# rubencart/NES-img-captioning

Hardware: AMD Instinct MI355X
Metric: population-members evaluated/sec (fc_caption, pop=512) at 1/2/4/8 GPUs (higher is better)
Workload: dtype fp32

## Files before the change

include/nicnes.h:

```cpp
#ifndef NICNES_H
#define NICNES_H

#include <stdint.h>

#ifdef __cplusplus
extern "C" {
#endif

#define NICNES_OK 0
#define NICNES_ERR_INVALID 1
#define NICNES_ERR_UNSUPPORTED 2
#define NICNES_ERR_HIP 3
#define NICNES_ERR_NOMEM 4
#define NICNES_ERR_FAULT 5

typedef struct nicnes_handle nicnes_handle;

typedef struct nicnes_config {
    int32_t vocab_size;
    int32_t input_encoding_size;
    int32_t rnn_size;
    int32_t fc_feat_size;
    int32_t seq_length;
    int32_t max_batch;
// ... 111 lines not shown
int nicnes_set_timing(nicnes_handle* h, int on);
int nicnes_kernel_times(nicnes_handle* h, float* out2_host);

int nicnes_decode_phase_times(nicnes_handle* h, float* out8_host);

int nicnes_set_decode_split(nicnes_handle* h, int32_t S, int32_t G);
int nicnes_decode_shape(nicnes_handle* h, int32_t B, int32_t count, int32_t* out3_host);
int nicnes_set_decode_streams(nicnes_handle* h, int32_t n);
int nicnes_set_decode_coop(nicnes_handle* h, int32_t mode);

int nicnes_sum_sensitivity(nicnes_handle* h, int32_t rows, float underflow, float* out_dev, void* stream);
int nicnes_decode_path(nicnes_handle* h, int32_t B, int32_t count, int32_t* out_host);
int nicnes_last_decode_lse(nicnes_handle* h, int32_t* bounded_host);
int nicnes_set_decode_screen(nicnes_handle* h, int32_t mode);
int nicnes_screen_stats(nicnes_handle* h, int64_t* out2_host);
int nicnes_test_logit_chain(nicnes_handle* h, uint64_t iteration, int32_t member, float sigma, int32_t sign,
                            const float* h_rows_dev, float* out_mfma_dev, float* out_chain_dev, void* stream);
int nicnes_test_certify_items(nicnes_handle* h, uint64_t iteration, int32_t member, float sigma, int32_t sign,
                              const float* h_rows_dev, const int32_t* items_host, int32_t n_items, float* out_dev,
                              void* stream);
int nicnes_test_certify_items_owned(nicnes_handle* h, uint64_t iteration, int32_t member, float sigma, int32_t sign,
                                    int32_t owner_by_id, const float* h_rows_dev, const int32_t* items_host,
                                    int32_t n_items, float* out_dev, void* stream);
int nicnes_test_score_rows(nicnes_handle* h, const int32_t* seq_dev, int32_t n_cand, int32_t rows,
                           const int32_t* member_batch_host, const float* lp_dev, const double* base_dev,
                           double* scores_out_dev, double* fitness_out_dev, void* stream);

int nicnes_es_create(nicnes_handle* h, int32_t max_parents, int32_t max_elites);
int nicnes_es_free(nicnes_handle* h);
int nicnes_es_set_mutation(nicnes_handle* h, int32_t mode);
// ... 27 lines not shown
```

nes-img-captioning_amd/csrc/decode_kernel.h:

```cpp
#pragma once
#define SCR_SLOTS (64 + 64 + 64 + 1 + 64)
#define PART_FLOATS (8 * 7 * 64)
#define COOP_CTR_STRIDE 32
#define SCREEN_CAP_WORDS(V1) ((size_t)(((V1) + 63) / 64) * 512)
#include <hip/hip_runtime.h>
#include <stdint.h>

struct DecodeParams {
    const float* theta;
    const float* noise;
    const uint64_t* noise_idx;
    const float* fc;
    const int32_t* member_batch;
    int32_t* seq;
    float* lp;
    const double* sample_u;
    float* scratch;
    int32_t* stats;
    float* slog;
    int32_t* slog_slots;
    int32_t slog_ns;
    int32_t* alive;
    int32_t* alive2;
    float* part;
// ... 10 lines not shown
    int32_t B_img;
    int32_t sign_off;
    int32_t rpi;
    int32_t G;
    int32_t S;
    int32_t alive_stride;
    int64_t D;
    int64_t off_img_w, off_img_b, off_emb_w, off_log_w, off_log_b, off_i2h_w, off_i2h_b, off_h2h_w, off_h2h_b;
};

struct ScreenArgs {
    uint32_t* cap;
    float* norm;
    float scale;
    unsigned long long* ctr;
};

struct MutHead {
    const float* head_noise;
    const uint64_t* head_idx;
    const float* mut_vec;
    int32_t mode;
};

struct ParentArgs {
    const float* parents;
    const int32_t* parent_of;
    int64_t stride;
};

#define DK_IMG 0
// ... 26 lines not shown
```

nes-img-captioning_amd/csrc/decode_kernel.hip:

```cpp
#include <hip/hip_runtime.h>
#include <stdint.h>

#include "../../include/nicnes_math.h"
#include "decode_kernel.h"

typedef float f32x4 __attribute__((ext_vector_type(4)));
typedef float f32x16 __attribute__((ext_vector_type(16)));
typedef unsigned u32x4 __attribute__((ext_vector_type(4)));
typedef __bf16 bf16x4 __attribute__((ext_vector_type(4)));
typedef __bf16 bf16x8 __attribute__((ext_vector_type(8)));
typedef __amdgpu_buffer_rsrc_t rsrc_t;

#define NTHREADS 512
#define LDS_ROW 132
#define SIGN_FLOATS (32 * LDS_ROW)
#define STAGE_FLOATS (2 * SIGN_FLOATS + 64)
#define STAGE64_FLOATS (2 * 64 * LDS_ROW + 128)
#define BF_ROW 68
#define BF_SIGN (64 * BF_ROW)
#define LOG2E 1.44269504088896340736f
#define H_SLOT_BYTES (4u * 64u * 64u)
#define NEG_INF (-__builtin_inff())

#ifndef DECODE_ABLATE
// ... 276 lines not shown
                                                const Stage64Regs& r) {
    float* b = buf + o.so;
#pragma unroll
    for (int u = 0; u < 4; ++u) {
        const f32x4 delta = r.z[u];
        *reinterpret_cast<f32x4*>(b + 16 * u * LDS_ROW) = r.w[u] + delta;
        *reinterpret_cast<f32x4*>(b + (64 + 16 * u) * LDS_ROW) = r.w[u] - delta;
    }
    if (bias) {
        const float delta = r.bz;
        const float v = o.bslot >= 64 ? r.bw - delta : r.bw + delta;
        buf[2 * 64 * LDS_ROW + o.bslot] = (o.bslot & 63) < valid ? v : NEG_INF;
    }
}

__device__ __forceinline__ void mfma_stage64(const float* w, const float* bias, const float (&Bop)[64], int lane,
                                             f32x16& acc0, f32x16& acc1) {
    const int hh = lane >> 5;
    const float* row0 = w + (lane & 31) * LDS_ROW + hh * 16;
    const float* row1 = row0 + 32 * LDS_ROW;
    acc0 = bias_init(bias, hh);
    acc1 = bias_init(bias + 32, hh);
#pragma unroll
    for (int T = 0; T < 4; ++T) {
        f32x4 a0[4], a1[4];
#pragma unroll
        for (int c = 0; c < 4; ++c) {
            a0[c] = *reinterpret_cast<const f32x4*>(row0 + T * 32 + 4 * c);
            a1[c] = *reinterpret_cast<const f32x4*>(row1 + T * 32 + 4 * c);
        }
// ... 697 lines not shown
    float acc = sgn ? bw - bz : bw + bz;
#pragma unroll
    for (int T = 0; T < 4; ++T) {
#pragma unroll
        for (int c = 0; c < 4; ++c) {
            const uint32_t ko = 4u * (uint32_t)(32 * T + 8 * c);
            const f32x4 w0 = ld4(theta_r, wo + ko), z0 = ld4(noise_r, wo + ko);
            const f32x4 w1 = ld4(theta_r, wo + ko + 16u), z1 = ld4(noise_r, wo + ko + 16u);
            const f32x4 a0 = sgn ? w0 - z0 : w0 + z0, a1 = sgn ? w1 - z1 : w1 + z1;
            acc = chain_chunk(acc, a0, a1, scr_r, row_lo, T, c);
        }
    }
    return acc;
}

__device__ __forceinline__ bool screen_scan(rsrc_t cap, uint32_t vo, int nst, float thr, float* lds, int tid, int& cnt,
                                            int& ncand) {
    uint32_t* list = reinterpret_cast<uint32_t*>(lds) + tid * SCREEN_HIT_CAP;
    int hits = 0;
    cnt = 0;
    for (int s0 = 0; s0 < nst; s0 += 16) {
        uint32_t wd[16];
#pragma unroll
        for (int j = 0; j < 16; ++j)
            wd[j] = __builtin_amdgcn_raw_buffer_load_b32(cap, (int)vo, (int)(2048u * (uint32_t)min(s0 + j, nst - 1)), 0);
#pragma unroll
        for (int j = 0; j < 16; ++j) {
            const uint32_t word = wd[j];
            if (s0 + j < nst && __builtin_bit_cast(float, word & ~31u) >= thr) {
                hits += (word & 16u) ? 4 : 1;
                ncand += (word & 16u) ? 32 : 2;
                if (cnt < SCREEN_HIT_CAP) list[cnt] = ((uint32_t)(s0 + j) << 8) | (word & 31u);
                ++cnt;
            }
        }
    }
    return hits <= SCREEN_HIT_CAP;
}

struct ListItems {
    const uint32_t* list;
    int cnt, hh, V1;
    template <class F>
    __device__ __forceinline__ void operator()(F&& f) const {
        for (int k = 0; k < cnt; ++k) {
            const uint32_t e = list[k];
            const int s = (int)(e >> 8), pr = (int)(e & 15u);
            const bool crowded = (e & 16u) != 0;
            const int i0 = crowded ? 0 : 2 * pr, i1 = crowded ? 32 : 2 * pr + 2;
            for (int i = i0; i < i1; ++i) {
                const int a = i & 15;
                const int v = 64 * s + 32 * (i >> 4) + 4 * hh + (a & 3) + 8 * (a >> 2);
// ... 37 lines not shown
__device__ __forceinline__ void cert_load_bias(const DecodeParams& p, rsrc_t theta_r, rsrc_t noise_r, const uint32_t* iw,
                                               int nv, float& bw, float& bz) {
    const uint32_t v = iw[min(lane_fresh() & 31, nv - 1)] & CERT_ID_MASK;
    const uint32_t bo = 4u * ((uint32_t)p.off_log_b + v);
    bw = ld1(theta_r, bo);
    bz = ld1(noise_r, bo);
}
__device__ __forceinline__ void cert_store(float* tile, int sgn, int T, const CertRegs& r) {
    const int lane = lane_fresh(), q = lane & 7;
    float* b = tile + (lane >> 3) * LDS_ROW + T * 32 + (q & 1) * 16 + 4 * (q >> 1);
#pragma unroll
    for (int u = 0; u < 4; ++u)
        *reinterpret_cast<f32x4*>(b + 8 * u * LDS_ROW) = sgn ? r.w[u] - r.z[u] : r.w[u] + r.z[u];
}

template <class Each, class Sink>
__device__ __forceinline__ void certify_tiles(const DecodeParams& p, rsrc_t theta_r, rsrc_t noise_r, int sgn,
                                              const float (&hB)[64], float* lds, int tid, int n_mine, const Each& each,
                                              Sink&& sink, int pm) {
    const int lane = tid & 63, hh = lane >> 5;
    const int wave = __builtin_amdgcn_readfirstlane(tid >> 6);
    float* tile = lds + CERT_WAVE_AT + wave * CERT_WAVE_FLOATS;
    float* bias = tile + SIGN_FLOATS;
    uint32_t* items = reinterpret_cast<uint32_t*>(bias + 32);
    int inc = n_mine;
#pragma unroll
    for (int d = 1; d < 64; d <<= 1) {
        const int u = __shfl_up(inc, d);
        inc += lane >= d ? u : 0;
    }
    const int total = __builtin_amdgcn_readlane(inc, 63), first = inc - n_mine;
    __syncthreads();
#if DECODE_PROF
    if (pm >= 0 && total == 0 && lane == 0)
        p.seq[(size_t)(blockIdx.x * gridDim.y + blockIdx.y) * 4096 + CERT_PROF_WAVE_AT((pm - 1 - 640) / 5 - 1) + wave] = 0;
#endif
    for (int b0 = 0; b0 < total; b0 += CERT_ITEMS) {
        const int nb = min(CERT_ITEMS, total - b0);
        const bool mine = first < b0 + nb && first + n_mine > b0;
        if (mine) {
            int pos = first - b0;
            each([&](int v) {
                if ((unsigned)pos < (unsigned)nb) items[pos] = ((uint32_t)lane << CERT_ID_BITS) | (uint32_t)v;
                ++pos;
            });
        }
        wave_lds_order();
// ... 65 lines not shown
    }
}

__global__ __launch_bounds__(NTHREADS) void nicnes_screen_norm_kernel(DecodeParams p, ScreenArgs sa) {
    __shared__ float red[4][8];
#include "screen_norm_body.inc"
}

__global__ __launch_bounds__(NTHREADS) void nicnes_screen_norm_es_kernel(DecodeParams p0, ParentArgs pa, ScreenArgs sa) {
    __shared__ float red[4][8];
    DecodeParams p = p0;
    p.theta = pa.parents + (int64_t)pa.parent_of[blockIdx.x] * pa.stride;
#include "screen_norm_body.inc"
}

template <int G, bool PAIRS, bool PEEL = true, class Tail = NoTail, class Hook = NoHook>
__device__ __forceinline__ void logit_stages(float* lds, const DecodeParams& p, uint64_t nidx, int wave, int sgn,
                                             int hf, const float (&hB)[64], int s0, int s1, RowState& st,
                                             Stage64Regs& s64, bool preloaded = false, Tail&& tail = Tail(),
                                             const Hook& hook = Hook()) {
    const rsrc_t lw_r = make_rsrc(p.theta + p.off_log_w, 4u * 128u * (uint32_t)p.V1);
    const rsrc_t lz_r = make_rsrc(p.noise + nidx + p.off_log_w, 4u * 128u * (uint32_t)p.V1);
    const rsrc_t lbw_r = make_rsrc(p.theta + p.off_log_b, 4u * (uint32_t)p.V1);
    const rsrc_t lbz_r = make_rsrc(p.noise + nidx + p.off_log_b, 4u * (uint32_t)p.V1);
    auto lsrc = [&](int s) {
        StageSrc Sx;
        Sx.w_r = lw_r; Sx.z_r = lz_r; Sx.b_r = lbw_r; Sx.bz_r = lbz_r;
        Sx.so_a = 32768u * (uint32_t)s; Sx.so_b = Sx.so_a + 16384u;
        Sx.bso = 256u * (uint32_t)s; Sx.bda = 0u; Sx.bdb = 128u;
        Sx.valid = p.V1 - 64 * s;
        return Sx;
    };
    const LaneOffs lo = lane_offs(wave, 128u);
    LaneOffsBf lob{0, 0};
    if constexpr (Hook::bf) lob = lane_offs_bf(wave);
    const int hh = lane_fresh() >> 5, vl = 4 * hh + (G == 4 ? 0 : 32 * hf);
    const bool bias = wave < 2;
    if (!preloaded) stage64_load_o(lsrc(s0), lo, bias, s64);
    auto sstore = [&](float* buf, int valid) __attribute__((always_inline)) {
        if constexpr (Hook::bf) stage64_store_bf(buf, valid, lo, lob.sob, bias, s64);
        else stage64_store_o(buf, valid, lo, bias, s64);
    };
    sstore(lds, lsrc(s0).valid);
    if (PEEL) stage64_load_o(lsrc(min(s0 + 1, s1 - 1)), lo, bias, s64);
    else if (s0 + 1 < s1) stage64_load_o(lsrc(s0 + 1), lo, bias, s64);
    __syncthreads();
    f32x16 a0, a1, b0, b1;
#pragma unroll
    for (int r = 0; r < 16; ++r) { b0[r] = NEG_INF; b1[r] = NEG_INF; }
    auto stage = [&](auto mode_t, int s, f32x16& o0, f32x16& o1, const f32x16& q0, const f32x16& q1) {
        constexpr int MODE = decltype(mode_t)::value;
        const int sn = min(s + 1, s1 - 1);
        const float* buf = lds + ((s - s0) & 1) * STAGE64_FLOATS;
        const float* wsg = buf + sgn * (Hook::bf ? BF_SIGN : 64 * LDS_ROW);
        const float* bsg = buf + 2 * (Hook::bf ? BF_SIGN : 64 * LDS_ROW) + 64 * sgn;
        auto mid = [&]() __attribute__((always_inline)) {
#if !(DECODE_ABLATE & 2)
            if constexpr (MODE == 0) {
                sstore(lds + ((s - s0 + 1) & 1) * STAGE64_FLOATS, lsrc(sn).valid);
                stage64_load_o(lsrc(min(s + 2, s1 - 1)), lo, bias, s64);
            } else if constexpr (MODE == 1) {
// ... 286 lines not shown
            for (int i = 0; i < 64; ++i) Bb[i >> 3][i & 7] = (__bf16)hB[i];
            const ScreenStage ss{scap_r, 4u * (uint32_t)(c.wave * 64 + lane_fresh()), 2.0f * seps + SCREEN_HU_MAX, Bb, st};
            logit_stages<4, true, true>(lds, p, nidx, c.wave, c.sgn, 0, hB, 0, nl, st, s64, pre, tail, ss);
        } else {
            logit_stages<4, PAIRS>(lds, p, nidx, c.wave, c.sgn, 0, hB, 0, nl, st, s64, pre, tail);
        }
        cell_pre = xpre;
        PROF_MARK(120 + 24 * (t + 1));

        const float m_o = __shfl_xor(st.m, 32);
        const float s_o = __shfl_xor(st.s, 32);
        float m = fmaxf(st.m, m_o);
        float stot = st.s * __builtin_amdgcn_exp2f((st.m - m) * LOG2E) + s_o * __builtin_amdgcn_exp2f((m_o - m) * LOG2E);
        TieWindow w = tie_window(stot, PAIRS, SCREEN ? p.lse_margin + 2.0f * seps : p.lse_margin);
        bool sforce = false;
        float lse = w.lse;
        int tok = 0x7fffffff;
        float lp_tok = 0.f;
        bool amb = false;
        if constexpr (SAMPLE) {
            const double u = u_pre;
            const float mo = __shfl_xor(sm, 32), ro = __shfl_xor(sref, 32);
            const double To = __shfl_xor(sT, 32);
            const float mr = fmaxf(sm, mo), R = fmaxf(sref, ro);
            const double ta = samp_scale(sT, sref - R), tb = samp_scale(To, ro - R);
            const double T = c.hh == 0 ? ta + tb : tb + ta;
            const float lse_s = (float)(log(T) + (double)R * 0.69314718055994531 - (double)mr);
            const uint32_t vo = 16u * (uint32_t)c.lane + SLOG_WAVE_BYTES * (uint32_t)c.wave;
#if DECODE_ABLATE & 512
            tok = 1 + (int)(u * 9000.0);
            lp_tok = -lse_s;
#else
            if (p.force_exact)
                sample_pick<true>(p, c.slog_r, vo, c.hh, mr, lse_s, R, u * T, tok, lp_tok);
            else
                sample_pick<false>(p, c.slog_r, vo, c.hh, mr, lse_s, R, u * T, tok, lp_tok, 120 + 24 * (t + 1));
#endif
        } else {
            if constexpr (SCREEN) {
                const float d = 2.0f * seps + w.hu_out;
                const float thr = (m - d) - SCREEN_PACK_REL * (fabsf(m) + d);
                const bool need = unf_prev != 0.f || p.no_mask;
                bool bad = p.force_exact || !(fabsf(thr) < 3.0e38f) || !(w.hu_out <= SCREEN_HU_MAX) || !(stot > 0.f);
                st.r1v = st.r0v = st.ev = NEG_INF;
                st.r1i = st.r0i = 0x7fffffff;
                int ncand = 0, ccnt = 0;
                if (need && !bad) {
                    bad = !screen_scan(scap_r, 4u * (uint32_t)(c.wave * 64 + lane_fresh()), nl, thr, lds,
                                       c.wave * 64 + lane_fresh(), ccnt, ncand);
                    if (bad) ccnt = 0;
                }
                PROF_MARK(CERT_PROF_AT(t));
                {
                    const int ctid = c.wave * 64 + lane_fresh();
                    const ListItems items{reinterpret_cast<const uint32_t*>(lds) + ctid * SCREEN_HIT_CAP, ccnt, c.hh, p.V1};
                    int n_mine = 0;
                    items([&](int) { ++n_mine; });
                    certify_tiles(p, c.theta_r, c.noise_r, c.sgn, hB, lds, ctid, n_mine, items,
                                  [&](float L, int v) { record1(st, L, v); }, CERT_PROF_AT(t) + 1);
                }
                PROF_MARK(CERT_PROF_AT(t) + 4);
#pragma unroll
                for (int dd = 32; dd >= 1; dd >>= 1) ncand += __shfl_xor(ncand, dd);
                if (ncand && lane_fresh() == 0) atomicAdd(sa->ctr, (unsigned long long)ncand);
                const float mx = fmaxf(st.r1v, __shfl_xor(st.r1v, 32));
                const float sv[4] = {st.r0v, st.r1v, __shfl_xor(st.r0v, 32), __shfl_xor(st.r1v, 32)};
                const int si[4] = {st.r0i, st.r1i, __shfl_xor(st.r0i, 32), __shfl_xor(st.r1i, 32)};
                int stok = 0x7fffffff;
                bool und = win_state(st.ev, mx, w) != 0 || win_state(__shfl_xor(st.ev, 32), mx, w) != 0;
#pragma unroll
                for (int k = 0; k < 4; ++k) {
                    const int ws = win_state(sv[k], mx, w);
                    if (ws == 1 && si[k] < stok) stok = si[k];
                    und = und || ws == 2;
                }
                const bool bad_o = __shfl_xor((int)bad, 32) != 0;
                bad = need && (bad || und || bad_o);
                if (bad && c.hh == 0) atomicAdd(sa->ctr + 1, 1ull);
                sforce = __syncthreads_or(bad ? 1 : 0) != 0;
                if (!sforce) {
                    tok = stok;
                } else {
                    row_state_init(st);
                    logit_stages<4, true>(lds, p, nidx, c.wave, c.sgn, 0, hB, 0, nl, st, s64, false);
                    cell_pre = false;
                    const float m2 = __shfl_xor(st.m, 32), s2 = __shfl_xor(st.s, 32);
                    m = fmaxf(st.m, m2);
                    stot = st.s * __builtin_amdgcn_exp2f((st.m - m) * LOG2E) + s2 * __builtin_amdgcn_exp2f((m2 - m) * LOG2E);
                    w = tie_window(stot, true, p.lse_margin);
                    lse = w.lse;
                }
            }
            if (!SCREEN || sforce) {
            const float cv[4] = {st.r0v, st.r1v, __shfl_xor(st.r0v, 32), __shfl_xor(st.r1v, 32)};
            const int ci[4] = {st.r0i, st.r1i, __shfl_xor(st.r0i, 32), __shfl_xor(st.r1i, 32)};
#pragma unroll
            for (int k = 0; k < 4; ++k) {
                const int ws = win_state(cv[k], m, w);
                if (ws == 1 && ci[k] < tok) tok = ci[k];
                amb = amb || ws == 2;
            }
        const bool ovf = p.force_exact || amb || win_state(st.ev, m, w) != 0 ||
                         win_state(__shfl_xor(st.ev, 32), m, w) != 0;
        if (__syncthreads_or(ovf ? 1 : 0)) {
            int best = 0x7fffffff;
            float ssum = 0.f;
            bool find = true;
            if (PAIRS) {
                exact_sweep(lds, p, c.theta_r, c.noise_r, c.tid, c.sgn, c.hh, c.lane, hB, true, true, m, 0.f,
                            ssum, best);
                lse = logf(ssum + __shfl_xor(ssum, 32));
                const float cv[4] = {st.r0v, st.r1v, __shfl_xor(st.r0v, 32), __shfl_xor(st.r1v, 32)};
                const int ci[4] = {st.r0i, st.r1i, __shfl_xor(st.r0i, 32), __shfl_xor(st.r1i, 32)};
                int t2 = 0x7fffffff;
#pragma unroll
                for (int k = 0; k < 4; ++k)
                    if (in_window(cv[k], m, lse) && ci[k] < t2) t2 = ci[k];
                const bool ev2 = p.force_exact || in_window(st.ev, m, lse) || in_window(__shfl_xor(st.ev, 32), m, lse);
                find = __syncthreads_or(ev2 ? 1 : 0) != 0;
                if (!find) tok = t2;
            }
            if (find) {
                exact_sweep(lds, p, c.theta_r, c.noise_r, c.tid, c.sgn, c.hh, c.lane, hB, true, false, m, lse,
                            ssum, best);
                tok = min(best, __shfl_xor(best, 32));
            }
            if (c.tid == 0) atomicAdd(p.stats + 0, 1);
        }
            }
        lp_tok = -lse;
        }
        if (tok >= p.V1) tok = 0;
        const bool unfinished = unf_prev != 0.f && tok > 0;
        it = (unfinished || p.no_mask) ? tok : 0;
        st1(c.scr_r, lo, U_SLOT, unfinished ? 1.f : 0.f);
#if !DECODE_PROF
        if (c.hh == 0 && c.row_valid) {
            const size_t o = (((size_t)c.member * 2 + c.sgn) * p.B + c.b) * p.T + (t - 1);
            p.seq[o] = it;
            if (p.lp) p.lp[o] = lp_tok;
        }
#endif
// ... 1370 lines not shown
```

nes-img-captioning_amd/csrc/engine.cpp:

```cpp
#include <hip/hip_runtime.h>

#include <cmath>
#include <cstdio>
#include <cstdlib>
#include <cstring>
#include <string>
#include <vector>
#include <algorithm>

#include <rccl/rccl.h>

#include "../../include/nicnes.h"
#include "../../include/nicnes_math.h"
#include "cider_kernel.h"
#include "decode_kernel.h"
#include "update_kernels.h"
#include "sensitivity.h"

#define SCREEN_DEFAULT 2
#define MB_RING 4

struct nicnes_handle {
    nicnes_config cfg;
    int device = 0;
// ... 102 lines not shown

    ncclComm_t comm = nullptr;
    bool comm_owned = false;
    int comm_nranks = 1;

    bool timing = false;
    int force_exact = 0;
    float lse_margin = 2e-3f;
    int bounded_mode = 2;
    int screen_mode = SCREEN_DEFAULT;
    float screen_scale = 1.0f;
    uint32_t* screen_cap = nullptr;
    int64_t screen_wgs = 0;
    float* screen_norm = nullptr;
    unsigned long long* screen_ctr = nullptr;
    int exact_left = 0;
    int last_bounded = 0;
    int last_decode_bounded = 0;
    int32_t fb_seen = 0;
    int32_t* stats_host = nullptr;
    hipEvent_t stats_ev = nullptr;
    bool stats_pending = false;
    hipEvent_t ev[3] = {nullptr, nullptr, nullptr};
    hipEvent_t dev[DECODE_MAX_EVENTS] = {};
    int dev_kind[DECODE_MAX_EVENTS] = {};
    int n_dev = 0;
    bool multi_stream = false;
    bool last_nes_form = true;
    bool step_pending_check = false;
    int64_t t_prev = 0;
// ... 144 lines not shown
    *nslabs = nslabs_of(B, *G);
    *S = h->dec_S ? h->dec_S : auto_split((int64_t)count * *nslabs, h->n_cu, *G);
}

bool coop_fits(const nicnes_handle* h, int G, int nslabs, int S, int count) {
    return h->coop_mode && G == 4 && (S == 2 || S == 4) && (h->V1 + 63) / 64 >= S &&
           (int64_t)count * nslabs * S <= (int64_t)h->coop_occ * h->n_cu;
}

void ensure_screen(nicnes_handle* h) {
    if (!h->screen_mode || (h->screen_cap && h->screen_norm)) return;
    const int64_t wgs = (int64_t)h->cfg.max_members * nslabs_of(h->cfg.max_batch, 4);
    bool ok = hipMalloc((void**)&h->screen_cap, (size_t)wgs * SCREEN_CAP_WORDS(h->V1) * sizeof(uint32_t)) == hipSuccess;
    if (ok) ok = hipMalloc((void**)&h->screen_norm, (size_t)h->cfg.max_members * 4 * sizeof(float)) == hipSuccess;
    if (ok && !h->screen_ctr)
        ok = hipMalloc((void**)&h->screen_ctr, 2 * sizeof(unsigned long long)) == hipSuccess &&
             hipMemset(h->screen_ctr, 0, 2 * sizeof(unsigned long long)) == hipSuccess;
    if (ok) {
        h->screen_wgs = wgs;
        return;
    }
    (void)hipGetLastError();
    if (h->screen_cap) (void)hipFree(h->screen_cap);
    if (h->screen_norm) (void)hipFree(h->screen_norm);
    h->screen_cap = nullptr;
    h->screen_norm = nullptr;
    h->screen_mode = 0;
}

int alloc_refs(nicnes_handle* h, int max_refs) {
    void* old[] = {h->ref_keys, h->ref_vec, h->ref_count, h->ref_len2, h->ref_norm};
    for (void* q : old)
// ... 112 lines not shown
        if (ds && ds[0] >= '1' && ds[0] <= '4' && ds[1] == 0) h->dec_streams = ds[0] - '0';
        const char* dc = getenv("NICNES_DECODE_COOP");
        if (dc && (dc[0] == '0' || dc[0] == '1') && dc[1] == 0) h->coop_mode = dc[0] - '0';
        const char* cl = getenv("NICNES_COOP_LAUNCH");
        if (cl && (cl[0] == '0' || cl[0] == '1') && cl[1] == 0) h->coop_launch = cl[0] - '0';
        const char* st = getenv("NICNES_TEST_COOP_STALL");
        if (st && st[0]) h->test_stall_ms = (uint32_t)atoi(st);
        const char* sl = getenv("NICNES_TEST_COOP_STALL_LAUNCHES");
        if (sl && sl[0]) h->test_stall_left = atoi(sl);
        const char* ts = getenv("NICNES_TEST_SLOTS");
        if (ts && ts[0]) h->test_slots = atoi(ts);
        const char* sc = getenv("NICNES_SCREEN");
        if (sc && sc[0] >= '0' && sc[0] <= '2' && sc[1] == 0) h->screen_mode = sc[0] - '0';
        const char* se = getenv("NICNES_SCREEN_EPS_SCALE");
        if (se && se[0]) h->screen_scale = std::max(1.0f, (float)atof(se));
    }
    {
        int ncu = 0;
        if (hipDeviceGetAttribute(&ncu, hipDeviceAttributeMultiprocessorCount, device) == hipSuccess && ncu > 0)
            h->n_cu = ncu;
    }
    if (!rc && nicnes_decode_init() != hipSuccess) rc = fail(h, NICNES_ERR_HIP, "nicnes_decode_init");
    if (!rc && (nicnes_decode_occupancy(&h->coop_occ, &h->sample_occ) != hipSuccess || h->coop_occ < 1 ||
                h->sample_occ < 1))
        rc = fail(h, NICNES_ERR_HIP, "nicnes_decode_occupancy");
    if (!rc) rc = dalloc(h, &h->stats, 4);
    if (!rc && hipHostMalloc((void**)&h->stats_host, 4 * sizeof(int32_t), hipHostMallocDefault) != hipSuccess)
        rc = fail(h, NICNES_ERR_HIP, "hipHostMalloc");
    if (!rc && hipEventCreateWithFlags(&h->stats_ev, hipEventDisableTiming) != hipSuccess)
        rc = fail(h, NICNES_ERR_HIP, "hipEventCreate");
// ... 571 lines not shown
            const int nst = (h->V1 + 63) / 64;
            const size_t per = (size_t)nst * 18432 + (size_t)((nst + 7) / 8) * 2048;
            HIPC(h, hipDeviceSynchronize());
            int rc = dalloc(h, &h->slog, per * ns);
            if (!rc) rc = dalloc(h, &h->slog_slots, (size_t)ns);
            if (rc) return rc;
            HIPC(h, hipMemset(h->slog_slots, 0, ns * sizeof(int32_t)));
            h->slog_ns = ns;
        }
        p.slog = h->slog;
        p.slog_slots = h->slog_slots;
        p.slog_ns = h->slog_ns;
    }
    if ((int64_t)count * nslabs * S > h->part_cap)
        return fail(h, NICNES_ERR_INVALID, "decode split beyond the partial-state buffer (nicnes_set_decode_split)");
    ScreenArgs sa{nullptr, nullptr, h->screen_scale, h->screen_ctr};
    const bool screen_on = h->screen_mode == 1 || (h->screen_mode == 2 && (int64_t)count * nslabs >= h->n_cu);
    if (screen_on && !sampled && !p.lp && bounded && G == 4 && S == 1 && !(h->mut_mode && !eval_theta)) {
        if (h->screen_cap && h->screen_norm && (int64_t)count * nslabs <= h->screen_wgs) {
            sa.cap = h->screen_cap;
            sa.norm = h->screen_norm;
        }
    }
    p.G = G;
    p.S = S;
    p.part = h->part;
    p.coop = !sampled && coop_fits(h, G, nslabs, S, count) ? 1 : 0;
    p.coop_launch = h->coop_launch;
    if (!eval_theta && h->mut_mode) {
        const bool head = !sampled && !p.coop && G == 4 && S == 1 && !h->mut_full;
        const int64_t j0 = head ? h->off[3] : 0;
// ... 259 lines not shown
    p.sample_u = nullptr;
    p.slog = nullptr;
    p.slog_slots = nullptr;
    p.slog_ns = 0;
    p.scratch = sp->scratch;
    p.stats = h->stats;
    p.alive = sp->alive;
    p.alive_stride = 2 * sp->pm_cap;
    p.alive2 = sp->alive + p.alive_stride;
    p.part = sp->part;
    p.coop_ctr = sp->coop_ctr;
    p.force_exact = h->force_exact;
    p.lse_margin = h->lse_margin;
    const bool bounded = h->bounded_mode == 1 || (h->bounded_mode == 2 && h->exact_left == 0);
    p.bounded_lse = bounded ? 1 : 0;
    ScreenArgs sa{nullptr, nullptr, h->screen_scale, h->screen_ctr};
    const bool screen_on = h->screen_mode == 1 || (h->screen_mode == 2 && (int64_t)n_pm * nslabs >= h->n_cu);
    if (screen_on && !p.lp && bounded && G == 4 && S == 1 && h->screen_cap && h->screen_norm &&
        (int64_t)n_pm * nslabs <= h->screen_wgs && n_pm <= h->cfg.max_members) {
        sa.cap = h->screen_cap;
        sa.norm = h->screen_norm;
    }
    p.G = G;
    p.S = S;
    p.coop = coop_fits(h, G, nslabs, S, n_pm) ? 1 : 0;
    p.coop_launch = h->coop_launch;
    p.test_stall_ms = 0;
    p.no_exit = 0;
    p.no_mask = 0;
    p.B = SPLIT_ROWS;
    p.B_img = per;
// ... 292 lines not shown
    HIPC(h, hipMemcpy(st, h->stats, sizeof st, hipMemcpyDeviceToHost));
    for (int i = 0; i < 4; ++i) out4_host[i] = st[i];
    return NICNES_OK;
}

int nicnes_screen_stats(nicnes_handle* h, int64_t* out2_host) {
    if (!h || !out2_host) return NICNES_ERR_INVALID;
    unsigned long long st[2] = {0, 0};
    HIPC(h, hipSetDevice(h->device));
    if (h->screen_ctr) HIPC(h, hipMemcpy(st, h->screen_ctr, sizeof st, hipMemcpyDeviceToHost));
    out2_host[0] = (int64_t)st[0];
    out2_host[1] = (int64_t)st[1];
    return NICNES_OK;
}

int nicnes_set_decode_screen(nicnes_handle* h, int32_t mode) {
    if (!h || mode < 0 || mode > 2) return NICNES_ERR_INVALID;
    HIPC(h, hipSetDevice(h->device));
    h->screen_mode = mode;
    ensure_screen(h);
    return NICNES_OK;
}

int nicnes_set_timing(nicnes_handle* h, int on) {
    if (!h) return NICNES_ERR_INVALID;
    HIPC(h, hipSetDevice(h->device));
    if (on && !h->ev[0])
    {
        for (auto& e : h->ev) HIPC(h, hipEventCreate(&e));
        for (auto& e : h->dev) HIPC(h, hipEventCreate(&e));
// ... 703 lines not shown
    p.force_exact = h->force_exact;
    p.lse_margin = h->lse_margin;
    if (h->stats_pending && hipEventQuery(h->stats_ev) == hipSuccess) {
        const int32_t fb = h->stats_host[0];
        if (h->stats_host[2] != 0 || h->stats_host[3] != 0)
            return fail(h, NICNES_ERR_FAULT, "a decode on this handle lost rows (nicnes_stats, nicnes_clear_faults)");
        if (h->last_bounded && fb - h->fb_seen >= 2) h->exact_left = 32;
        h->fb_seen = fb;
        h->stats_pending = false;
    }
    const bool bounded = h->bounded_mode == 1 || (h->bounded_mode == 2 && h->exact_left == 0);
    if (h->bounded_mode == 2 && h->exact_left > 0 && !p.lp) --h->exact_left;
    p.bounded_lse = bounded ? 1 : 0;
    h->last_decode_bounded = (bounded && !p.lp) ? 1 : 0;
    const int rows = h->B, nslabs = nslabs_of(rows, 4);
    ScreenArgs sa{nullptr, nullptr, h->screen_scale, h->screen_ctr};
    const bool screen_on = h->screen_mode == 1 || (h->screen_mode == 2 && (int64_t)count * nslabs >= h->n_cu);
    if (!coop_S && screen_on && !p.lp && bounded && h->screen_cap && h->screen_norm &&
        (int64_t)count * nslabs <= h->screen_wgs) {
        sa.cap = h->screen_cap;
        sa.norm = h->screen_norm;
    }
    p.G = 4;
    p.S = coop_S ? coop_S : 1;
    p.part = h->part;
    p.coop = coop_S ? 1 : 0;
    p.coop_launch = h->coop_launch;
    p.test_stall_ms = h->test_stall_left != 0 ? h->test_stall_ms : 0;
    if (p.coop && h->test_stall_ms && h->test_stall_left > 0) --h->test_stall_left;
    p.no_exit = (p.lp && nslabs > 1) ? 1 : 0;
    p.coop_ctr = h->coop_ctr;
// ... 66 lines not shown
```

nes-img-captioning_amd/nicnes/_lib.py:

```python
import ctypes
import os

HERE = os.path.dirname(os.path.abspath(__file__))
LIB_PATH = os.path.join(HERE, 'libnicnes.so')

OK, ERR_INVALID, ERR_UNSUPPORTED, ERR_HIP, ERR_NOMEM, ERR_FAULT = 0, 1, 2, 3, 4, 5
COMM_ID_BYTES = 128
_NAMES = {ERR_INVALID: 'invalid argument', ERR_UNSUPPORTED: 'not supported', ERR_HIP: 'HIP error',
          ERR_NOMEM: 'out of device memory', ERR_FAULT: 'contained decode fault'}

EXPORTS = ['nicnes_param_count', 'nicnes_param_offsets', 'nicnes_create', 'nicnes_destroy', 'nicnes_last_error',
           'nicnes_set_noise_table', 'nicnes_set_theta', 'nicnes_get_theta', 'nicnes_set_adam_state',
           'nicnes_get_adam_state', 'nicnes_set_batch', 'nicnes_set_df_table', 'nicnes_noise_indices',
           'nicnes_evaluate', 'nicnes_rank_weights', 'nicnes_grad_partial', 'nicnes_adam_step', 'nicnes_stats',
           'nicnes_set_timing', 'nicnes_kernel_times', 'nicnes_decode_phase_times', 'nicnes_sgd_step',
           'nicnes_optimizer_update', 'nicnes_last_ratio', 'nicnes_set_fitness_mode', 'nicnes_evaluate_lp',
           'nicnes_set_decode_split', 'nicnes_decode_shape', 'nicnes_set_decode_streams', 'nicnes_comm_unique_id', 'nicnes_comm_init',
           'nicnes_comm_attach', 'nicnes_comm_destroy', 'nicnes_comm_count', 'nicnes_clear_faults', 'nicnes_allgather_fitness', 'nicnes_allreduce_grad',
           'nicnes_noise_vectors', 'nicnes_set_batches', 'nicnes_evaluate_batches', 'nicnes_set_mutation',
           'nicnes_set_mutation_proportional', 'nicnes_theta_zeros',
           'nicnes_set_decode_coop', 'nicnes_decode_path', 'nicnes_sum_sensitivity', 'nicnes_grad_partial_range',
           'nicnes_evaluate_theta', 'nicnes_set_sample_draws', 'nicnes_set_rows_per_image',
           'nicnes_last_decode_lse', 'nicnes_test_logit_chain', 'nicnes_test_score_rows',
           'nicnes_test_certify_items', 'nicnes_test_certify_items_owned',
           'nicnes_set_decode_screen', 'nicnes_screen_stats', 'nicnes_split_create', 'nicnes_split_destroy',
           'nicnes_split_decode', 'nicnes_split_score', 'nicnes_split_evaluate',
           'nicnes_es_create', 'nicnes_es_free', 'nicnes_es_set_mutation', 'nicnes_es_set_parent',
           'nicnes_es_set_parent_count', 'nicnes_es_get_row', 'nicnes_es_row_stats', 'nicnes_es_evaluate',
           'nicnes_es_offspring', 'nicnes_es_select', 'nicnes_es_advance', 'nicnes_es_set_elite',
           'nicnes_es_load_theta', 'nicnes_set_decode_es', 'nicnes_decode_path_es', 'nicnes_allgather_fitness_es']


class NicnesConfig(ctypes.Structure):
    _fields_ = [('vocab_size', ctypes.c_int32), ('input_encoding_size', ctypes.c_int32),
                ('rnn_size', ctypes.c_int32), ('fc_feat_size', ctypes.c_int32), ('seq_length', ctypes.c_int32),
                ('max_batch', ctypes.c_int32), ('max_refs', ctypes.c_int32), ('max_members', ctypes.c_int32),
                ('noise_len', ctypes.c_uint64), ('noise_seed', ctypes.c_uint64)]


class NicnesError(RuntimeError):
# ... 49 lines not shown
        'nicnes_grad_partial': (c.c_int, [vp, u64, i32, i32, vp, f32, vp, vp]),
        'nicnes_grad_partial_range': (c.c_int, [vp, u64, i32, i32, vp, f32, i64, i64, vp, vp]),
        'nicnes_adam_step': (c.c_int, [vp, vp, i32, f64, f64, f64, f64, f64, vp, vp]),
        'nicnes_stats': (c.c_int, [vp, vp]),
        'nicnes_set_timing': (c.c_int, [vp, c.c_int]),
        'nicnes_kernel_times': (c.c_int, [vp, vp]),
        'nicnes_decode_phase_times': (c.c_int, [vp, vp]),
        'nicnes_set_decode_split': (c.c_int, [vp, i32, i32]),
        'nicnes_decode_shape': (c.c_int, [vp, i32, i32, vp]),
        'nicnes_set_decode_streams': (c.c_int, [vp, i32]),
        'nicnes_set_decode_coop': (c.c_int, [vp, i32]),
        'nicnes_decode_path': (c.c_int, [vp, i32, i32, vp]),
        'nicnes_last_decode_lse': (c.c_int, [vp, vp]),
        'nicnes_set_decode_screen': (c.c_int, [vp, i32]),
        'nicnes_screen_stats': (c.c_int, [vp, vp]),
        'nicnes_test_logit_chain': (c.c_int, [vp, u64, i32, f32, i32, vp, vp, vp, vp]),
        'nicnes_test_certify_items': (c.c_int, [vp, u64, i32, f32, i32, vp, vp, i32, vp, vp]),
        'nicnes_test_certify_items_owned': (c.c_int, [vp, u64, i32, f32, i32, i32, vp, vp, i32, vp, vp]),
        'nicnes_test_score_rows': (c.c_int, [vp, vp, i32, i32, vp, vp, vp, vp, vp, vp]),
        'nicnes_sum_sensitivity': (c.c_int, [vp, i32, f32, vp, vp]),
        'nicnes_split_create': (c.c_int, [vp, vp, i32, vp, i32, vp, vp, vp, i64, f64, c.POINTER(vp), vp]),
        'nicnes_split_destroy': (c.c_int, [vp, vp]),
        'nicnes_split_decode': (c.c_int, [vp, vp, i32, i32, vp, vp, vp]),
        'nicnes_split_score': (c.c_int, [vp, vp, i32, i32, vp, vp, vp, vp, vp]),
        'nicnes_split_evaluate': (c.c_int, [vp, vp, i32, i32, vp, vp, vp, vp, vp]),
        'nicnes_es_create': (c.c_int, [vp, i32, i32]),
        'nicnes_es_free': (c.c_int, [vp]),
        'nicnes_es_set_mutation': (c.c_int, [vp, i32]),
        'nicnes_es_set_parent': (c.c_int, [vp, i32, vp, vp]),
        'nicnes_es_set_parent_count': (c.c_int, [vp, i32]),
# ... 40 lines not shown
```

nes-img-captioning_amd/nicnes/engine.py:

```python
import ctypes
import os

import numpy as np
import torch

from . import _lib
from ._lib import NicnesConfig, check

SEQ_LENGTH = 16


def pack_ngram(tokens):
    n = len(tokens)
    assert 1 <= n <= 4
    key = n << 56
    for k, t in enumerate(tokens):
        t = int(t)
        assert 0 <= t < 16384
        key |= t << (42 - 14 * k)
    return key


def df_table_arrays(document_frequency):
    items = sorted((pack_ngram(tuple(int(w) for w in g)), float(v)) for g, v in document_frequency.items())
# ... 539 lines not shown
        with torch.cuda.device(self.device):
            check(self.L.nicnes_allreduce_grad(self.h, _ptr(gsum), self._stream()), self.h, 'allreduce_grad')
        return gsum

    def clear_faults(self):
        out = (ctypes.c_int64 * 2)()
        with torch.cuda.device(self.device):
            check(self.L.nicnes_clear_faults(self.h, out), self.h, 'clear_faults')
        return {'coop_timeouts': int(out[0]), 'sample_slot_timeouts': int(out[1])}

    def stats(self):
        out = (ctypes.c_int64 * 4)()
        check(self.L.nicnes_stats(self.h, out), self.h, 'stats')
        sc = (ctypes.c_int64 * 2)()
        check(self.L.nicnes_screen_stats(self.h, sc), self.h, 'screen_stats')
        return {'tie_fallbacks': out[0], 'sample_stage_fallbacks': out[1], 'coop_timeouts': out[2],
                'sample_slot_timeouts': out[3], 'screen_candidates': sc[0], 'screen_fallback_rows': sc[1]}


METRIC_KEYS = ('Bleu_1', 'Bleu_2', 'Bleu_3', 'Bleu_4', 'ROUGE_L', 'CIDEr')


class Split:

    def __init__(self, engine, fc, gts=None, df=None, ref_len_raw=None):
        from .validation import corpus_df
        e = self.engine = engine
        T = e.cfg.seq_length
        fc_np = fc.detach().cpu().numpy() if isinstance(fc, torch.Tensor) else np.asarray(fc)
        fc_np = np.ascontiguousarray(fc_np, np.float32)
        if fc_np.ndim != 2 or fc_np.shape[1] != e.cfg.fc_feat_size or fc_np.shape[0] < 1:
            raise ValueError('fc must be [N >= 1, fc_feat_size]')
# ... 103 lines not shown
```

Measured before the change: 21390.

## Add multi-round screen certification and restrict exact fallback sweep to failing waves

When a row's screen hit list overflows the LDS cap, candidates are now processed over several certification rounds (up to a configurable limit) instead of forcing a full exact logit sweep. When a fallback sweep is still needed, only the waves (sign halves) that failed do the MFMA work; the others just keep the staging pipeline and barriers in step, and rows that already settled keep their screened token. This is meant to cut the cost of full-vocabulary fallback sweeps. It also adds more per-reason atomic counters and a stats API, which adds some atomic traffic and extra control flow.

```diff
diff --git a/include/nicnes.h b/include/nicnes.h
--- a/include/nicnes.h
+++ b/include/nicnes.h
@@ -149,6 +149,7 @@
 int nicnes_last_decode_lse(nicnes_handle* h, int32_t* bounded_host);
 int nicnes_set_decode_screen(nicnes_handle* h, int32_t mode);
 int nicnes_screen_stats(nicnes_handle* h, int64_t* out2_host);
+int nicnes_screen_reasons(nicnes_handle* h, int64_t* out16_host);
 int nicnes_test_logit_chain(nicnes_handle* h, uint64_t iteration, int32_t member, float sigma, int32_t sign,
                             const float* h_rows_dev, float* out_mfma_dev, float* out_chain_dev, void* stream);
 int nicnes_test_certify_items(nicnes_handle* h, uint64_t iteration, int32_t member, float sigma, int32_t sign,
diff --git a/nes-img-captioning_amd/csrc/decode_kernel.h b/nes-img-captioning_amd/csrc/decode_kernel.h
--- a/nes-img-captioning_amd/csrc/decode_kernel.h
+++ b/nes-img-captioning_amd/csrc/decode_kernel.h
@@ -48,7 +48,11 @@
     float* norm;
     float scale;
     unsigned long long* ctr;
+    int32_t rounds;
 };
+#define SCREEN_CTR_WORDS 18
+#define SCREEN_ROUNDS_DEFAULT 2
+#define SCREEN_ROUNDS_MAX 64
 
 struct MutHead {
     const float* head_noise;
diff --git a/nes-img-captioning_amd/csrc/decode_kernel.hip b/nes-img-captioning_amd/csrc/decode_kernel.hip
--- a/nes-img-captioning_amd/csrc/decode_kernel.hip
+++ b/nes-img-captioning_amd/csrc/decode_kernel.hip
@@ -314,6 +314,24 @@
     }
 }
 
+__device__ __forceinline__ void stage64_store_g(float* buf, int valid, const LaneOffs& o, bool bias,
+                                                const Stage64Regs& r, int signs) {
+    float* b = buf + o.so;
+    if (signs & 1) {
+#pragma unroll
+        for (int u = 0; u < 4; ++u) *reinterpret_cast<f32x4*>(b + 16 * u * LDS_ROW) = r.w[u] + r.z[u];
+    }
+    if (signs & 2) {
+#pragma unroll
+        for (int u = 0; u < 4; ++u) *reinterpret_cast<f32x4*>(b + (64 + 16 * u) * LDS_ROW) = r.w[u] - r.z[u];
+    }
+    if (bias) {
+        const float delta = r.bz;
+        const float v = o.bslot >= 64 ? r.bw - delta : r.bw + delta;
+        buf[2 * 64 * LDS_ROW + o.bslot] = (o.bslot & 63) < valid ? v : NEG_INF;
+    }
+}
+
 __device__ __forceinline__ void mfma_stage64(const float* w, const float* bias, const float (&Bop)[64], int lane,
                                              f32x16& acc0, f32x16& acc1) {
     const int hh = lane >> 5;
@@ -1041,12 +1059,13 @@
     return acc;
 }
 
-__device__ __forceinline__ bool screen_scan(rsrc_t cap, uint32_t vo, int nst, float thr, float* lds, int tid, int& cnt,
-                                            int& ncand) {
+__device__ __forceinline__ void screen_scan(rsrc_t cap, uint32_t vo, int nst, float thr, float* lds, int tid, bool first,
+                                            int from, int& cnt, int& next, int& hits, int& ncand) {
     uint32_t* list = reinterpret_cast<uint32_t*>(lds) + tid * SCREEN_HIT_CAP;
-    int hits = 0;
+    int wsum = 0;
     cnt = 0;
-    for (int s0 = 0; s0 < nst; s0 += 16) {
+    next = nst;
+    for (int s0 = from; s0 < nst && (first || next == nst); s0 += 16) {
         uint32_t wd[16];
 #pragma unroll
         for (int j = 0; j < 16; ++j)
@@ -1055,14 +1074,22 @@
         for (int j = 0; j < 16; ++j) {
             const uint32_t word = wd[j];
             if (s0 + j < nst && __builtin_bit_cast(float, word & ~31u) >= thr) {
-                hits += (word & 16u) ? 4 : 1;
-                ncand += (word & 16u) ? 32 : 2;
-                if (cnt < SCREEN_HIT_CAP) list[cnt] = ((uint32_t)(s0 + j) << 8) | (word & 31u);
-                ++cnt;
-            }
-        }
-    }
-    return hits <= SCREEN_HIT_CAP;
+                const int wt = (word & 16u) ? 4 : 1;
+                if (first) {
+                    hits += wt;
+                    ncand += (word & 16u) ? 32 : 2;
+                }
+                if (next == nst) {
+                    if (wsum + wt <= SCREEN_HIT_CAP) {
+                        list[cnt++] = ((uint32_t)(s0 + j) << 8) | (word & 31u);
+                        wsum += wt;
+                    } else {
+                        next = s0 + j;
+                    }
+                }
+            }
+        }
+    }
 }
 
 struct ListItems {
@@ -1130,7 +1157,7 @@
         *reinterpret_cast<f32x4*>(b + 8 * u * LDS_ROW) = sgn ? r.w[u] - r.z[u] : r.w[u] + r.z[u];
 }
 
-template <class Each, class Sink>
+template <bool SYNC = true, class Each, class Sink>
 __device__ __forceinline__ void certify_tiles(const DecodeParams& p, rsrc_t theta_r, rsrc_t noise_r, int sgn,
                                               const float (&hB)[64], float* lds, int tid, int n_mine, const Each& each,
                                               Sink&& sink, int pm) {
@@ -1146,7 +1173,7 @@
         inc += lane >= d ? u : 0;
     }
     const int total = __builtin_amdgcn_readlane(inc, 63), first = inc - n_mine;
-    __syncthreads();
+    if constexpr (SYNC) __syncthreads();
 #if DECODE_PROF
     if (pm >= 0 && total == 0 && lane == 0)
         p.seq[(size_t)(blockIdx.x * gridDim.y + blockIdx.y) * 4096 + CERT_PROF_WAVE_AT((pm - 1 - 640) / 5 - 1) + wave] = 0;
@@ -1242,11 +1269,12 @@
 #include "screen_norm_body.inc"
 }
 
-template <int G, bool PAIRS, bool PEEL = true, class Tail = NoTail, class Hook = NoHook>
+template <int G, bool PAIRS, bool PEEL = true, class Tail = NoTail, class Hook = NoHook, bool GATED = false>
 __device__ __forceinline__ void logit_stages(float* lds, const DecodeParams& p, uint64_t nidx, int wave, int sgn,
                                              int hf, const float (&hB)[64], int s0, int s1, RowState& st,
                                              Stage64Regs& s64, bool preloaded = false, Tail&& tail = Tail(),
-                                             const Hook& hook = Hook()) {
+                                             const Hook& hook = Hook(), bool gact = true, int gsgn = 3) {
+    static_assert(!GATED || (G == 4 && !Hook::bf), "the gated loop is the fp32 64-row loop");
     const rsrc_t lw_r = make_rsrc(p.theta + p.off_log_w, 4u * 128u * (uint32_t)p.V1);
     const rsrc_t lz_r = make_rsrc(p.noise + nidx + p.off_log_w, 4u * 128u * (uint32_t)p.V1);
     const rsrc_t lbw_r = make_rsrc(p.theta + p.off_log_b, 4u * (uint32_t)p.V1);
@@ -1267,12 +1295,27 @@
     if (!preloaded) stage64_load_o(lsrc(s0), lo, bias, s64);
     auto sstore = [&](float* buf, int valid) __attribute__((always_inline)) {
         if constexpr (Hook::bf) stage64_store_bf(buf, valid, lo, lob.sob, bias, s64);
+        else if constexpr (GATED) stage64_store_g(buf, valid, lo, bias, s64, gsgn);
         else stage64_store_o(buf, valid, lo, bias, s64);
     };
     sstore(lds, lsrc(s0).valid);
     if (PEEL) stage64_load_o(lsrc(min(s0 + 1, s1 - 1)), lo, bias, s64);
     else if (s0 + 1 < s1) stage64_load_o(lsrc(s0 + 1), lo, bias, s64);
     __syncthreads();
+    if constexpr (GATED) {
+        if (!gact) {
+            for (int s = s0; s < s1; ++s) {
+                if (s + 1 < s1) {
+                    sstore(lds + ((s - s0 + 1) & 1) * STAGE64_FLOATS, lsrc(s + 1).valid);
+                    if (s + 2 < s1) stage64_load_o(lsrc(s + 2), lo, bias, s64);
+                } else {
+                    tail();
+                }
+                __syncthreads();
+            }
+            return;
+        }
+    }
     f32x16 a0, a1, b0, b1;
 #pragma unroll
     for (int r = 0; r < 16; ++r) { b0[r] = NEG_INF; b1[r] = NEG_INF; }
@@ -1589,6 +1632,8 @@
         float stot = st.s * __builtin_amdgcn_exp2f((st.m - m) * LOG2E) + s_o * __builtin_amdgcn_exp2f((m_o - m) * LOG2E);
         TieWindow w = tie_window(stot, PAIRS, SCREEN ? p.lse_margin + 2.0f * seps : p.lse_margin);
         bool sforce = false;
+        bool sact = true;
+        int stok = 0x7fffffff;
         float lse = w.lse;
         int tok = 0x7fffffff;
         float lp_tok = 0.f;
@@ -1616,23 +1661,36 @@
                 const float d = 2.0f * seps + w.hu_out;
                 const float thr = (m - d) - SCREEN_PACK_REL * (fabsf(m) + d);
                 const bool need = unf_prev != 0.f || p.no_mask;
-                bool bad = p.force_exact || !(fabsf(thr) < 3.0e38f) || !(w.hu_out <= SCREEN_HU_MAX) || !(stot > 0.f);
+                const bool pre = p.force_exact || !(fabsf(thr) < 3.0e38f) || !(w.hu_out <= SCREEN_HU_MAX) || !(stot > 0.f);
                 st.r1v = st.r0v = st.ev = NEG_INF;
                 st.r1i = st.r0i = 0x7fffffff;
-                int ncand = 0, ccnt = 0;
-                if (need && !bad) {
-                    bad = !screen_scan(scap_r, 4u * (uint32_t)(c.wave * 64 + lane_fresh()), nl, thr, lds,
-                                       c.wave * 64 + lane_fresh(), ccnt, ncand);
-                    if (bad) ccnt = 0;
-                }
-                PROF_MARK(CERT_PROF_AT(t));
-                {
-                    const int ctid = c.wave * 64 + lane_fresh();
+                const int ctid = c.wave * 64 + lane_fresh();
+                const uint32_t cvo = 4u * (uint32_t)ctid;
+                int ncand = 0, hits = 0, nxt = nl;
+                bool over = false, multi = false;
+                auto round = [&](int ccnt, int pm) __attribute__((always_inline)) {
                     const ListItems items{reinterpret_cast<const uint32_t*>(lds) + ctid * SCREEN_HIT_CAP, ccnt, c.hh, p.V1};
                     int n_mine = 0;
                     items([&](int) { ++n_mine; });
-                    certify_tiles(p, c.theta_r, c.noise_r, c.sgn, hB, lds, ctid, n_mine, items,
-                                  [&](float L, int v) { record1(st, L, v); }, CERT_PROF_AT(t) + 1);
+                    certify_tiles<false>(p, c.theta_r, c.noise_r, c.sgn, hB, lds, ctid, n_mine, items,
+                                         [&](float L, int v) { record1(st, L, v); }, pm);
+                };
+                {
+                    int ccnt = 0;
+                    if (need && !pre) screen_scan(scap_r, cvo, nl, thr, lds, ctid, true, 0, ccnt, nxt, hits, ncand);
+                    PROF_MARK(CERT_PROF_AT(t));
+                    over = hits > SCREEN_HIT_CAP;
+                    const int ov = __ockl_wgred_or_i32((over ? 1 : 0) | (hits > SCREEN_HIT_CAP * max(sa->rounds, 1) ? 2 : 0));
+                    multi = ov == 1;
+                    if (over && !multi) { ccnt = 0; nxt = nl; }
+                    round(ccnt, CERT_PROF_AT(t) + 1);
+                }
+                if (__builtin_expect(multi, 0)) {
+                    while (__syncthreads_or(nxt < nl ? 1 : 0)) {
+                        int ccnt = 0;
+                        if (nxt < nl) screen_scan(scap_r, cvo, nl, thr, lds, ctid, false, nxt, ccnt, nxt, hits, ncand);
+                        round(ccnt, -1);
+                    }
                 }
                 PROF_MARK(CERT_PROF_AT(t) + 4);
 #pragma unroll
@@ -1641,29 +1699,55 @@
                 const float mx = fmaxf(st.r1v, __shfl_xor(st.r1v, 32));
                 const float sv[4] = {st.r0v, st.r1v, __shfl_xor(st.r0v, 32), __shfl_xor(st.r1v, 32)};
                 const int si[4] = {st.r0i, st.r1i, __shfl_xor(st.r0i, 32), __shfl_xor(st.r1i, 32)};
-                int stok = 0x7fffffff;
-                bool und = win_state(st.ev, mx, w) != 0 || win_state(__shfl_xor(st.ev, 32), mx, w) != 0;
+                const bool evw = win_state(st.ev, mx, w) != 0 || win_state(__shfl_xor(st.ev, 32), mx, w) != 0;
+                bool und2 = false;
 #pragma unroll
                 for (int k = 0; k < 4; ++k) {
                     const int ws = win_state(sv[k], mx, w);
                     if (ws == 1 && si[k] < stok) stok = si[k];
-                    und = und || ws == 2;
+                    und2 = und2 || ws == 2;
                 }
-                const bool bad_o = __shfl_xor((int)bad, 32) != 0;
-                bad = need && (bad || und || bad_o);
-                if (bad && c.hh == 0) atomicAdd(sa->ctr + 1, 1ull);
-                sforce = __syncthreads_or(bad ? 1 : 0) != 0;
-                if (!sforce) {
-                    tok = stok;
-                } else {
-                    row_state_init(st);
-                    logit_stages<4, true>(lds, p, nidx, c.wave, c.sgn, 0, hB, 0, nl, st, s64, false);
+                const int hits_o = __shfl_xor(hits, 32);
+                const bool over_r = over || hits_o > SCREEN_HIT_CAP;
+                const bool pre_r = pre || __shfl_xor((int)pre, 32) != 0;
+                const bool bad1 = need && (pre_r || over_r || evw || und2);
+                const bool bad = need && (pre_r || (over_r && !multi) || evw || und2);
+                {
+                    auto rows = [&](bool f, int k) __attribute__((always_inline)) {
+                        const unsigned long long bl = __ballot(f && c.hh == 0);
+                        if (bl && lane_fresh() == 0) atomicAdd(sa->ctr + k, (unsigned long long)__popcll(bl));
+                    };
+                    rows(bad1, 1);
+                    if (__ballot(bad1)) {
+                        rows(bad1 && over_r, 2);
+                        rows(bad1 && und2, 3);
+                        rows(bad1 && evw, 4);
+                        rows(bad1 && pre_r, 5);
+                        rows(bad1 && !bad, 6);
+                        rows(bad, 7);
+                        const int hmax = max(hits, hits_o), hk = min((hmax + SCREEN_HIT_CAP - 1) / SCREEN_HIT_CAP, 9) - 2;
+                        for (int k = 0; k < 8; ++k) rows(need && over_r && hk == k, 9 + k);
+                    }
+                }
+                const int wbad = __ockl_wgred_or_i32(__ballot(bad) ? 1 << c.wave : 0);
+                sforce = wbad != 0;
+                sact = ((wbad >> c.wave) & 1) != 0;
+                if (sforce && c.tid == 0) atomicAdd(sa->ctr + 8, 1ull);
+                if (sact && lane_fresh() == 0) atomicAdd(sa->ctr + 17, 1ull);
+                if (!sact) tok = stok;
+                if (__builtin_expect(sforce, 0)) {
+                    const int sgn_on = ((wbad & 0x0f) ? 1 : 0) | ((wbad & 0xf0) ? 2 : 0);
+                    if (sact) row_state_init(st);
+                    logit_stages<4, true, true, NoTail, NoHook, true>(lds, p, nidx, c.wave, c.sgn, 0, hB, 0, nl, st, s64, false,
+                                                                      NoTail(), NoHook(), sact, sgn_on);
                     cell_pre = false;
-                    const float m2 = __shfl_xor(st.m, 32), s2 = __shfl_xor(st.s, 32);
-                    m = fmaxf(st.m, m2);
-                    stot = st.s * __builtin_amdgcn_exp2f((st.m - m) * LOG2E) + s2 * __builtin_amdgcn_exp2f((m2 - m) * LOG2E);
-                    w = tie_window(stot, true, p.lse_margin);
-                    lse = w.lse;
+                    if (sact) {
+                        const float m2 = __shfl_xor(st.m, 32), s2 = __shfl_xor(st.s, 32);
+                        m = fmaxf(st.m, m2);
+                        stot = st.s * __builtin_amdgcn_exp2f((st.m - m) * LOG2E) + s2 * __builtin_amdgcn_exp2f((m2 - m) * LOG2E);
+                        w = tie_window(stot, true, p.lse_margin);
+                        lse = w.lse;
+                    }
                 }
             }
             if (!SCREEN || sforce) {
@@ -1672,11 +1756,11 @@
 #pragma unroll
             for (int k = 0; k < 4; ++k) {
                 const int ws = win_state(cv[k], m, w);
-                if (ws == 1 && ci[k] < tok) tok = ci[k];
+                if (ws == 1 && ci[k] < tok && (!SCREEN || sact)) tok = ci[k];
                 amb = amb || ws == 2;
             }
-        const bool ovf = p.force_exact || amb || win_state(st.ev, m, w) != 0 ||
-                         win_state(__shfl_xor(st.ev, 32), m, w) != 0;
+        const bool ovf = (!SCREEN || sact) && (p.force_exact || amb || win_state(st.ev, m, w) != 0 ||
+                                               win_state(__shfl_xor(st.ev, 32), m, w) != 0);
         if (__syncthreads_or(ovf ? 1 : 0)) {
             int best = 0x7fffffff;
             float ssum = 0.f;
@@ -1691,7 +1775,8 @@
 #pragma unroll
                 for (int k = 0; k < 4; ++k)
                     if (in_window(cv[k], m, lse) && ci[k] < t2) t2 = ci[k];
-                const bool ev2 = p.force_exact || in_window(st.ev, m, lse) || in_window(__shfl_xor(st.ev, 32), m, lse);
+                const bool ev2 = (!SCREEN || sact) &&
+                                 (p.force_exact || in_window(st.ev, m, lse) || in_window(__shfl_xor(st.ev, 32), m, lse));
                 find = __syncthreads_or(ev2 ? 1 : 0) != 0;
                 if (!find) tok = t2;
             }
@@ -1701,6 +1786,7 @@
                 tok = min(best, __shfl_xor(best, 32));
             }
             if (c.tid == 0) atomicAdd(p.stats + 0, 1);
+            if (SCREEN && !sact) tok = stok;
         }
             }
         lp_tok = -lse;
diff --git a/nes-img-captioning_amd/csrc/engine.cpp b/nes-img-captioning_amd/csrc/engine.cpp
--- a/nes-img-captioning_amd/csrc/engine.cpp
+++ b/nes-img-captioning_amd/csrc/engine.cpp
@@ -140,6 +140,7 @@
     int64_t screen_wgs = 0;
     float* screen_norm = nullptr;
     unsigned long long* screen_ctr = nullptr;
+    int screen_rounds = SCREEN_ROUNDS_DEFAULT;
     int exact_left = 0;
     int last_bounded = 0;
     int last_decode_bounded = 0;
@@ -314,8 +315,8 @@
     bool ok = hipMalloc((void**)&h->screen_cap, (size_t)wgs * SCREEN_CAP_WORDS(h->V1) * sizeof(uint32_t)) == hipSuccess;
     if (ok) ok = hipMalloc((void**)&h->screen_norm, (size_t)h->cfg.max_members * 4 * sizeof(float)) == hipSuccess;
     if (ok && !h->screen_ctr)
-        ok = hipMalloc((void**)&h->screen_ctr, 2 * sizeof(unsigned long long)) == hipSuccess &&
-             hipMemset(h->screen_ctr, 0, 2 * sizeof(unsigned long long)) == hipSuccess;
+        ok = hipMalloc((void**)&h->screen_ctr, SCREEN_CTR_WORDS * sizeof(unsigned long long)) == hipSuccess &&
+             hipMemset(h->screen_ctr, 0, SCREEN_CTR_WORDS * sizeof(unsigned long long)) == hipSuccess;
     if (ok) {
         h->screen_wgs = wgs;
         return;
@@ -458,6 +459,8 @@
         if (sc && sc[0] >= '0' && sc[0] <= '2' && sc[1] == 0) h->screen_mode = sc[0] - '0';
         const char* se = getenv("NICNES_SCREEN_EPS_SCALE");
         if (se && se[0]) h->screen_scale = std::max(1.0f, (float)atof(se));
+        const char* sr = getenv("NICNES_SCREEN_ROUNDS");
+        if (sr && sr[0]) h->screen_rounds = std::min(SCREEN_ROUNDS_MAX, std::max(1, atoi(sr)));
     }
     {
         int ncu = 0;
@@ -1059,7 +1062,7 @@
     }
     if ((int64_t)count * nslabs * S > h->part_cap)
         return fail(h, NICNES_ERR_INVALID, "decode split beyond the partial-state buffer (nicnes_set_decode_split)");
-    ScreenArgs sa{nullptr, nullptr, h->screen_scale, h->screen_ctr};
+    ScreenArgs sa{nullptr, nullptr, h->screen_scale, h->screen_ctr, h->screen_rounds};
     const bool screen_on = h->screen_mode == 1 || (h->screen_mode == 2 && (int64_t)count * nslabs >= h->n_cu);
     if (screen_on && !sampled && !p.lp && bounded && G == 4 && S == 1 && !(h->mut_mode && !eval_theta)) {
         if (h->screen_cap && h->screen_norm && (int64_t)count * nslabs <= h->screen_wgs) {
@@ -1349,7 +1352,7 @@
     p.lse_margin = h->lse_margin;
     const bool bounded = h->bounded_mode == 1 || (h->bounded_mode == 2 && h->exact_left == 0);
     p.bounded_lse = bounded ? 1 : 0;
-    ScreenArgs sa{nullptr, nullptr, h->screen_scale, h->screen_ctr};
+    ScreenArgs sa{nullptr, nullptr, h->screen_scale, h->screen_ctr, h->screen_rounds};
     const bool screen_on = h->screen_mode == 1 || (h->screen_mode == 2 && (int64_t)n_pm * nslabs >= h->n_cu);
     if (screen_on && !p.lp && bounded && G == 4 && S == 1 && h->screen_cap && h->screen_norm &&
         (int64_t)n_pm * nslabs <= h->screen_wgs && n_pm <= h->cfg.max_members) {
@@ -1672,6 +1675,15 @@
     return NICNES_OK;
 }
 
+int nicnes_screen_reasons(nicnes_handle* h, int64_t* out16_host) {
+    if (!h || !out16_host) return NICNES_ERR_INVALID;
+    unsigned long long st[SCREEN_CTR_WORDS] = {0};
+    HIPC(h, hipSetDevice(h->device));
+    if (h->screen_ctr) HIPC(h, hipMemcpy(st, h->screen_ctr, sizeof st, hipMemcpyDeviceToHost));
+    for (int i = 2; i < SCREEN_CTR_WORDS; ++i) out16_host[i - 2] = (int64_t)st[i];
+    return NICNES_OK;
+}
+
 int nicnes_set_decode_screen(nicnes_handle* h, int32_t mode) {
     if (!h || mode < 0 || mode > 2) return NICNES_ERR_INVALID;
     HIPC(h, hipSetDevice(h->device));
@@ -2405,7 +2417,7 @@
     p.bounded_lse = bounded ? 1 : 0;
     h->last_decode_bounded = (bounded && !p.lp) ? 1 : 0;
     const int rows = h->B, nslabs = nslabs_of(rows, 4);
-    ScreenArgs sa{nullptr, nullptr, h->screen_scale, h->screen_ctr};
+    ScreenArgs sa{nullptr, nullptr, h->screen_scale, h->screen_ctr, h->screen_rounds};
     const bool screen_on = h->screen_mode == 1 || (h->screen_mode == 2 && (int64_t)count * nslabs >= h->n_cu);
     if (!coop_S && screen_on && !p.lp && bounded && h->screen_cap && h->screen_norm &&
         (int64_t)count * nslabs <= h->screen_wgs) {
diff --git a/nes-img-captioning_amd/nicnes/_lib.py b/nes-img-captioning_amd/nicnes/_lib.py
--- a/nes-img-captioning_amd/nicnes/_lib.py
+++ b/nes-img-captioning_amd/nicnes/_lib.py
@@ -23,7 +23,7 @@
            'nicnes_evaluate_theta', 'nicnes_set_sample_draws', 'nicnes_set_rows_per_image',
            'nicnes_last_decode_lse', 'nicnes_test_logit_chain', 'nicnes_test_score_rows',
            'nicnes_test_certify_items', 'nicnes_test_certify_items_owned',
-           'nicnes_set_decode_screen', 'nicnes_screen_stats', 'nicnes_split_create', 'nicnes_split_destroy',
+           'nicnes_set_decode_screen', 'nicnes_screen_stats', 'nicnes_screen_reasons', 'nicnes_split_create', 'nicnes_split_destroy',
            'nicnes_split_decode', 'nicnes_split_score', 'nicnes_split_evaluate',
            'nicnes_es_create', 'nicnes_es_free', 'nicnes_es_set_mutation', 'nicnes_es_set_parent',
            'nicnes_es_set_parent_count', 'nicnes_es_get_row', 'nicnes_es_row_stats', 'nicnes_es_evaluate',
@@ -103,6 +103,7 @@
         'nicnes_last_decode_lse': (c.c_int, [vp, vp]),
         'nicnes_set_decode_screen': (c.c_int, [vp, i32]),
         'nicnes_screen_stats': (c.c_int, [vp, vp]),
+        'nicnes_screen_reasons': (c.c_int, [vp, vp]),
         'nicnes_test_logit_chain': (c.c_int, [vp, u64, i32, f32, i32, vp, vp, vp, vp]),
         'nicnes_test_certify_items': (c.c_int, [vp, u64, i32, f32, i32, vp, vp, i32, vp, vp]),
         'nicnes_test_certify_items_owned': (c.c_int, [vp, u64, i32, f32, i32, i32, vp, vp, i32, vp, vp]),
diff --git a/nes-img-captioning_amd/nicnes/engine.py b/nes-img-captioning_amd/nicnes/engine.py
--- a/nes-img-captioning_amd/nicnes/engine.py
+++ b/nes-img-captioning_amd/nicnes/engine.py
@@ -577,8 +577,15 @@
         check(self.L.nicnes_stats(self.h, out), self.h, 'stats')
         sc = (ctypes.c_int64 * 2)()
         check(self.L.nicnes_screen_stats(self.h, sc), self.h, 'screen_stats')
-        return {'tie_fallbacks': out[0], 'sample_stage_fallbacks': out[1], 'coop_timeouts': out[2],
-                'sample_slot_timeouts': out[3], 'screen_candidates': sc[0], 'screen_fallback_rows': sc[1]}
+        sr = (ctypes.c_int64 * 16)()
+        check(self.L.nicnes_screen_reasons(self.h, sr), self.h, 'screen_reasons')
+        d = {'tie_fallbacks': out[0], 'sample_stage_fallbacks': out[1], 'coop_timeouts': out[2],
+             'sample_slot_timeouts': out[3], 'screen_candidates': sc[0], 'screen_fallback_rows': sc[1],
+             'screen_rows_over_cap': sr[0], 'screen_rows_undecided': sr[1], 'screen_rows_evicted': sr[2],
+             'screen_rows_nonfinite': sr[3], 'screen_rows_settled_later': sr[4], 'screen_resweep_rows': sr[5],
+             'screen_resweep_steps': sr[6], 'screen_resweep_waves': sr[15]}
+        d.update({'screen_over_cap_rounds_%d' % (k + 2): sr[7 + k] for k in range(8)})
+        return d
 
 
 METRIC_KEYS = ('Bleu_1', 'Bleu_2', 'Bleu_3', 'Bleu_4', 'ROUGE_L', 'CIDEr')
```

Result: faster. 24180 (median of 6 runs) (+13.0%).
